# BurntSushi/aho-corasick

Hardware: NVIDIA H100
Metric: haystack_scan_throughput (higher is better)
Workload: dtype u8

## Files before the change

### aho-corasick_b200/csrc/acb_api.cu

```cuda
#include <cuda_runtime.h>

#include <algorithm>
#include <chrono>
#include <cstdio>
#include <cstdlib>
#include <cstring>
#include <atomic>
#include <pthread.h>
#include <condition_variable>
#include <functional>
#include <mutex>
#include <thread>
#include <new>
#include <optional>
#include <vector>

#include "../../include/acb200.h"
#include "../../include/acb200_debug.h"
#include "acb_build.hpp"
#include "acb_comm.hpp"
#include "acb_device.cuh"
#include "acb_plan.hpp"

using acb::DfaDev;
// ... 324 lines not shown
  d.pattern_lens = a->d_plens;
  d.depth16 = a->d_depth16;
  d.stride2 = h.stride2;
  d.max_match_id = h.max_match_id;
  d.start_unanchored_id = h.start_unanchored_id;
  d.start_anchored_id = h.start_anchored_id;
  d.max_pattern_len = uint32_t(std::min<uint64_t>(h.max_pattern_len, UINT32_MAX));
  d.min_pattern_len = uint32_t(std::min<uint64_t>(h.min_pattern_len, UINT32_MAX));
  d.amap = a->d_amap;
  acb::plan_device_fields(a->pf, d);
  a->on_device = true;
  return ACG_OK;
}

int reserve_tuples(Workspace& w, uint64_t cap) {
  return reserve_all(cap, w.d_keys[0], w.d_pids[0], w.d_keys[1], w.d_pids[1]);
}

template <class F>
int cub_call(Workspace& w, F f) {
  size_t tb = 0;
  CK(f(nullptr, tb));
  int rc = w.d_temp.reserve(std::max<size_t>(tb, 16));
  if (rc) return rc;
  tb = w.d_temp.cap;
  CK(f(w.d_temp, tb));
  return ACG_OK;
}

int reserve_rec(Workspace& w, uint64_t n) {
  n = std::max<uint64_t>(n, 1 << 16) * 3;
  int rc = w.d_rec.reserve(n);
  return rc ? rc : w.h_rec.reserve(n);
}

int reserve_docs(Workspace& w, uint64_t n) {
  return reserve_all(std::max<uint64_t>(n, 1 << 12), w.d_doc_offs, w.d_doc_counts, w.d_doc_incl, w.d_doc_flags);
}

int check_anchored(int have, int want_anchored) {
  if (have == ACG_START_BOTH) return ACG_OK;
  if (have == ACG_START_UNANCHORED) return want_anchored ? ACG_E_INVALID_INPUT_ANCHORED : ACG_OK;
  return want_anchored ? ACG_OK : ACG_E_INVALID_INPUT_UNANCHORED;
}
bool span_ok(uint64_t hay_len, uint64_t s, uint64_t e) { return e <= hay_len && s <= e + 1; }
int check_start(const HostDfa& h, int anchored) {
  if (anchored) return h.start_anchored_id == 0 ? ACG_E_INVALID_INPUT_ANCHORED : ACG_OK;
  return h.start_unanchored_id == 0 ? ACG_E_INVALID_INPUT_UNANCHORED : ACG_OK;
}

struct TupleResult {
  uint64_t n = 0;
  int sorted_buf = 0;
};

struct DocBatch {
  const uint64_t* d_offsets = nullptr;
  uint64_t n = 0;
  bool unordered = false;
};

struct BucketPlan {
  uint32_t shift = 0;
  uint32_t n = 0, log = 0, tie_bits = 0;
  uint64_t slots() const { return uint64_t(n) << log; }
};

BucketPlan plan_buckets(const acg_dfa* a, uint64_t n_bytes) {
  BucketPlan b;
  if (a->experiment & ACG_EXP_GLOBAL_TILES) return b;
  const uint32_t tie_bits = uint32_t(acb::bit_width(a->h.max_pattern_len)) + a->pf.dup_shift;
  if (tie_bits >= 32) return b;
  const uint32_t max_shift = 32 - tie_bits;
  uint32_t shift = std::min<uint32_t>(25, max_shift);
  uint32_t min_shift = 22;
  uint32_t log = acb::kOrderLog;
#ifdef ACB_EMULATE
  if (const char* e = getenv("ACB_EMU_BUCKETSHIFT")) { shift = std::min<uint32_t>(uint32_t(atoi(e)), max_shift); min_shift = 1; }
  if (const char* e = getenv("ACB_EMU_BUCKETLOG")) log = std::min<uint32_t>(uint32_t(std::max(atoi(e), 0)), acb::kOrderLog);
#endif
  if (shift < min_shift) return b;
  while ((n_bytes >> shift) + 1 > acb::kMaxBuckets) {
    if (shift >= max_shift) return b;
    ++shift;
  }
  b.shift = shift;
  b.n = uint32_t((n_bytes >> shift) + 1);
  b.log = log;
  b.tie_bits = tie_bits;
  return b;
}

int enqueue_prefilter_range(const acg_dfa* a, const uint8_t* d_hay, uint64_t readable,
                            uint64_t span_start, uint64_t span_end, uint64_t scan_lo,
                            uint64_t scan_hi, int mode, int dev_sms, const BucketPlan& bp,
                            const DocBatch* docs) {
  Workspace& w = cur_ws();
  const acb::PrefilterPlan& pf = a->pf;
  const uintptr_t base = reinterpret_cast<uintptr_t>(d_hay);
  uint64_t lo = scan_lo + ((16 - ((base + scan_lo) & 15)) & 15);
  const uint64_t limit = std::min<uint64_t>(scan_hi, readable >= 20 ? readable - 20 : 0);
  uint64_t hi = lo;
  if (limit > lo) hi = lo + ((limit - lo) & ~15ull);
  if (lo > scan_hi) { lo = scan_hi; hi = scan_hi; }
  acb::PrefilterLaunch p;
  p.hay = d_hay;
  p.hay_len = readable;
  p.span_start = span_start;
  p.span_end = span_end;
  p.bitmap = a->d_bitmap;
  p.log_bits = pf.log_bits;
  p.k = pf.k;
  p.stride = pf.stride;
  p.geom = pf.wide ? 1 : 0;
  p.dyn = (a->experiment & ACG_EXP_STATIC_TILES) ? 0 : ((a->experiment & ACG_EXP_GLOBAL_TILES) ? 2 : 1);
  p.kmask = pf.kmask;
  p.fold = pf.fold;
  p.mult = pf.mult;
  p.mult3 = pf.mult3;
  p.key_shift = pf.key_shift;
  p.shift = pf.shift;
  p.dense = pf.dense ? 1 : 0;
  p.brute = pf.brute ? 1 : 0;
  p.mode = mode == 1 ? 1 : 0;
  p.first_only = mode == 2 ? 1 : 0;
  p.dup_shift = pf.dup_shift;
  p.scan_lo = scan_lo;
  p.scan_hi = scan_hi;
  p.region_lo = lo;
  p.region_hi = hi;
  p.keys = w.d_keys[0];
  p.pids = w.d_pids[0];
  p.counter = w.d_counter;
  p.cap = w.tuple_cap();
  p.bucket_shift = bp.shift;
  p.bucket_log = bp.log;
  p.bucket_slots = bp.slots();
  p.doc_offsets = docs ? docs->d_offsets : nullptr;
  p.n_docs = docs ? docs->n : 0;
  p.bs_n = 0;
  for (int i = 0; i < 3; ++i) { p.bs_needle[i] = 0; p.bs_back[i] = 0; }
  if (pf.bs_n && !a->bytescan_inert && !(a->experiment & ACG_EXP_NO_BYTESCAN)) {
    p.bs_n = pf.bs_n;
    for (uint32_t i = 0; i < pf.bs_n; ++i) { p.bs_needle[i] = uint32_t(pf.bs_byte[i]) * 0x01010101u; p.bs_back[i] = pf.bs_back[i]; }
    CK(acb::launch_bytescan(a->dev, p, dev_sms, w.stream));
  } else {
    if (p.dyn == 2) CK(cudaMemsetAsync(w.d_counter + 2, 0, 8, w.stream));
    CK(acb::launch_prefilter(a->dev, p, dev_sms, w.stream));
  }
  cur_ws().stats.launches += 1;
  return ACG_OK;
}

int order_tuples(const acg_dfa* a, uint64_t want, uint64_t n_bytes, TupleResult* res, const BucketPlan& bp,
                 uint64_t overflow) {
  Workspace& w = cur_ws();
  res->n = want;
  cur_ws().stats.raw_matches = want;
  res->sorted_buf = 0;
  if (want <= 1 && (bp.shift == 0 || want == 0)) return ACG_OK;
  const int end_bit = std::min(64, acb::kTieBits + acb::bit_width(n_bytes + 1));
  float ms = 0;
  CK(cudaEventRecord(w.ev2, w.stream));
  auto sort_list = [&](int from) {
    return cub_call(w, [&](void* t, size_t& tb) {
      return acb::sort_pairs(t, tb, w.d_keys[from], w.d_keys[1 - from], w.d_pids[from], w.d_pids[1 - from], want,
                             end_bit, w.stream);
    });
  };
  int rc;
  if (bp.shift == 0) {
    if ((rc = sort_list(0))) return rc;
    cur_ws().stats.launches += 8;
    res->sorted_buf = 1;
  } else {
    acb::OrderLaunch o;
    o.keys_in = w.d_keys[0];
    o.pids_in = w.d_pids[0];
    o.keys_out = w.d_keys[1];
    o.pids_out = w.d_pids[1];
    o.bucket_count = w.d_counter + acb::kBucketCountersAt;
    o.overflow_count = w.d_counter;
    o.n_buckets = bp.n;
    o.bucket_shift = bp.shift;
    o.bucket_cap = 1u << bp.log;
    o.tie_bits = bp.tie_bits;
    o.bucket_slots = bp.slots();
    if (overflow == 0) {
      CK(acb::launch_order_buckets(o, w.stream));
      cur_ws().stats.launches += 1;
      res->sorted_buf = 1;
    } else {
      CK(acb::launch_compact_buckets(o, w.stream));
      if ((rc = sort_list(1))) return rc;
      cur_ws().stats.launches += 9;
      res->sorted_buf = 0;
    }
  }
  CK(cudaEventRecord(w.ev3, w.stream));
  CK(cudaStreamSynchronize(w.stream));
  cudaEventElapsedTime(&ms, w.ev2, w.ev3);
  cur_ws().stats.order_ms = ms;
  return ACG_OK;
}

int run_walk_overlapping(const acg_dfa* a, const uint8_t* d_hay, uint64_t readable, uint64_t span_start,
                         uint64_t span_end, TupleResult* res) {
  Workspace& w = cur_ws();
  const uint64_t n_bytes = span_end - span_start;
  if (a->max_list_len >= (1u << acb::kTieBits)) return ACG_E_INVALID_ARG;
  if (n_bytes >= (1ull << (64 - acb::kTieBits))) return ACG_E_INVALID_ARG;
  int dev_sms = 132;
  cudaDeviceGetAttribute(&dev_sms, cudaDevAttrMultiProcessorCount, a->device);
  const uint64_t target_lanes = uint64_t(dev_sms) * 2048;
  uint64_t seg_len = (n_bytes + target_lanes - 1) / std::max<uint64_t>(target_lanes, 1);
  seg_len = std::max<uint64_t>(seg_len, 256);
  seg_len = (seg_len + 15) & ~15ull;
  const uint64_t n_segs = std::max<uint64_t>((n_bytes + seg_len - 1) / seg_len, 1);
  uint64_t cap = std::max<uint64_t>(w.tuple_cap(), std::max<uint64_t>(1 << 20, n_bytes / 256));
  for (int attempt = 0; attempt < 8; ++attempt) {
    int rc = reserve_tuples(w, cap);
    if (rc) return rc;
    CK(cudaMemsetAsync(w.d_counter, 0, 8, w.stream));
    acb::WalkLaunch p;
    p.hay = d_hay;
    p.hay_len = readable;
    p.span_start = span_start;
    p.span_end = span_end;
    p.seg_len = seg_len;
    p.n_segs = n_segs;
    p.keys = w.d_keys[0];
    p.pids = w.d_pids[0];
    p.counter = w.d_counter;
    p.cap = w.tuple_cap();
    CK(cudaEventRecord(w.ev0, w.stream));
    CK(acb::launch_walk_overlapping(a->dev, p, w.stream));
    CK(cudaEventRecord(w.ev1, w.stream));
    CK(cudaMemcpyAsync(w.h_counter, w.d_counter, 8, cudaMemcpyDeviceToHost, w.stream));
    CK(cudaStreamSynchronize(w.stream));
    cur_ws().stats.launches += 1;
    const uint64_t want = *w.h_counter;
    if (want > w.tuple_cap()) { cap = want + want / 8 + 1024; continue; }
    float ms = 0;
    cudaEventElapsedTime(&ms, w.ev0, w.ev1);
    cur_ws().stats.scan_ms = ms;
    return order_tuples(a, want, n_bytes, res, BucketPlan{}, 0);
  }
  return ACG_E_NOMEM;
}

class CopyPool {
 public:
  static CopyPool& get() {
    static std::once_flag once;
    std::call_once(once, [] { pthread_atfork(nullptr, nullptr, [] { instance().store(nullptr); }); });
    CopyPool* p = instance().load(std::memory_order_acquire);
    if (!p) {
      CopyPool* fresh = new CopyPool;
      if (instance().compare_exchange_strong(p, fresh)) p = fresh;
    }
    return *p;
  }
  void copy(uint8_t* dst, const uint8_t* src, size_t n) {
    if (n < (4u << 20) || workers_.empty()) { std::memcpy(dst, src, n); return; }
    std::unique_lock<std::mutex> lk(mu_);
    busy_cv_.wait(lk, [&] { return !active_; });
    active_ = true;
    dst_ = dst; src_ = src; n_ = n;
    next_.store(0);
    pending_ = int(workers_.size());
    ++epoch_;
    cv_.notify_all();
    done_cv_.wait(lk, [&] { return pending_ == 0; });
    active_ = false;
    busy_cv_.notify_one();
  }

 private:
  static std::atomic<CopyPool*>& instance() {
    static std::atomic<CopyPool*> p{nullptr};
    return p;
  }
  CopyPool() {
    unsigned n = std::thread::hardware_concurrency();
    n = n >= 16 ? 8 : (n >= 4 ? n / 2 : 0);
    for (unsigned i = 0; i < n; ++i) workers_.emplace_back([this] { run(); });
    for (auto& t : workers_) t.detach();
  }
  void run() {
    uint64_t seen = 0;
    for (;;) {
      std::unique_lock<std::mutex> lk(mu_);
      cv_.wait(lk, [&] { return epoch_ != seen; });
      seen = epoch_;
      uint8_t* dst = dst_;
      const uint8_t* src = src_;
      const size_t n = n_;
      lk.unlock();
      constexpr size_t kSlice = 1u << 20;
      for (;;) {
        const size_t off = next_.fetch_add(kSlice);
        if (off >= n) break;
        std::memcpy(dst + off, src + off, std::min(kSlice, n - off));
      }
      lk.lock();
      if (--pending_ == 0) done_cv_.notify_one();
    }
  }
  std::mutex mu_;
  std::condition_variable cv_, done_cv_, busy_cv_;
  std::vector<std::thread> workers_;
  uint8_t* dst_ = nullptr;
  const uint8_t* src_ = nullptr;
  size_t n_ = 0;
  std::atomic<size_t> next_{0};
  int pending_ = 0;
  uint64_t epoch_ = 0;
  bool active_ = false;
};

bool is_pageable_host(const void* p) {
  cudaPointerAttributes attr;
  if (cudaPointerGetAttributes(&attr, p) != cudaSuccess) { cudaGetLastError(); return false; }
  return attr.type == cudaMemoryTypeUnregistered;
}

int reserve_stage(Workspace& w, uint64_t bytes) {
  for (int i = 0; i < 2; ++i) {
    int rc = w.h_stage[i].reserve(bytes);
    if (rc) return rc;
    if (!w.stage_ev[i]) CK(cudaEventCreateWithFlags(&w.stage_ev[i], cudaEventDisableTiming));
  }
  return ACG_OK;
}

int run_prefilter(const acg_dfa* a, const uint8_t* d_hay, uint64_t readable, uint64_t span_start,
                  uint64_t span_end, int mode, TupleResult* res, const uint8_t* h_hay = nullptr,
                  uint64_t scan_lo = UINT64_MAX, uint64_t scan_hi = UINT64_MAX, const DocBatch* docs = nullptr) {
  if (scan_lo == UINT64_MAX) { scan_lo = span_start; scan_hi = span_end; }
  const bool unordered = docs && docs->unordered;
  Workspace& w = cur_ws();
  const uint64_t n_bytes = span_end - span_start;
  if (n_bytes >= (1ull << (64 - acb::kTieBits))) return ACG_E_INVALID_ARG;
  int dev_sms = 132;
  cudaDeviceGetAttribute(&dev_sms, cudaDevAttrMultiProcessorCount, a->device);
  uint64_t cap = std::max<uint64_t>(w.tuple_cap(), std::max<uint64_t>(1 << 20, (scan_hi - scan_lo) / 256));
  const BucketPlan bp = unordered ? BucketPlan{} : plan_buckets(a, n_bytes);
  cap = std::max<uint64_t>(cap, bp.slots() + (bp.shift ? (1u << 16) : 0));
  const size_t counter_bytes = bp.shift ? 8 * (acb::kBucketCountersAt + size_t(bp.n)) : 16;
  bool copied = h_hay == nullptr;
  for (int attempt = 0; attempt < 8; ++attempt) {
    int rc = reserve_tuples(w, cap);
    if (rc) return rc;
    CK(cudaMemsetAsync(w.d_counter, 0, counter_bytes, w.stream));
    CK(cudaEventRecord(w.ev0, w.stream));
    if (copied) {
      if ((rc = enqueue_prefilter_range(a, d_hay, readable, span_start, span_end, scan_lo, scan_hi, mode,
                                        dev_sms, bp, docs)))
        return rc;
    } else {
      const uint64_t chunk = a->pipeline_chunk;
      const uint64_t tail = std::min<uint64_t>(a->h.max_pattern_len, 1u << 30) + 64;
      uint64_t scanned = span_start;
      const bool staged = span_end - span_start >= std::min<uint64_t>(8u << 20, chunk) && is_pageable_host(h_hay + span_start);
      if (staged && (rc = reserve_stage(w, std::min<uint64_t>(chunk, span_end - span_start)))) return rc;
      bool stage_used[2] = {false, false};
      int stage_i = 0;
      CK(cudaEventRecord(w.ev2, w.copy_stream));
      for (uint64_t c0 = span_start; c0 < span_end; c0 += chunk) {
        const uint64_t c1 = std::min(span_end, c0 + chunk);
        const uint8_t* src = h_hay + c0;
        if (staged) {
          if (stage_used[stage_i]) CK(cudaEventSynchronize(w.stage_ev[stage_i]));
          CopyPool::get().copy(w.h_stage[stage_i], h_hay + c0, size_t(c1 - c0));
          src = w.h_stage[stage_i];
        }
        CK(cudaMemcpyAsync(const_cast<uint8_t*>(d_hay) + c0, src, c1 - c0, cudaMemcpyHostToDevice,
                           w.copy_stream));
        if (staged) {
          CK(cudaEventRecord(w.stage_ev[stage_i], w.copy_stream));
          stage_used[stage_i] = true;
          stage_i ^= 1;
        }
        CK(cudaEventRecord(w.ev3, w.copy_stream));
        CK(cudaStreamWaitEvent(w.stream, w.ev3, 0));
        const uint64_t upto = c1 == span_end ? span_end : (c1 > scanned + tail ? c1 - tail : scanned);
        if (upto > scanned || c1 == span_end) {
          if ((rc = enqueue_prefilter_range(a, d_hay, c1 == span_end ? readable : c1, span_start, span_end,
                                            scanned, upto, mode, dev_sms, bp, docs)))
            return rc;
          scanned = upto;
        }
      }
      copied = true;
    }
    CK(cudaEventRecord(w.ev1, w.stream));
    CK(cudaMemcpyAsync(w.h_counter, w.d_counter, counter_bytes, cudaMemcpyDeviceToHost, w.stream));
    CK(cudaStreamSynchronize(w.stream));
    uint64_t want = w.h_counter[0], overflow = 0, room = w.tuple_cap();
    if (bp.shift) {
      overflow = want;
      want = 0;
      for (uint32_t i = 0; i < bp.n; ++i) want += w.h_counter[acb::kBucketCountersAt + i];
      room = w.tuple_cap() - bp.slots();
    }
    cur_ws().stats.candidates = w.h_counter[1];
    if (a->pf.bs_n && !a->bytescan_inert && scan_hi - scan_lo >= (1u << 16) && w.h_counter[1] > (scan_hi - scan_lo) / 64)
      a->bytescan_inert = true;
    float ms = 0;
    cudaEventElapsedTime(&ms, w.ev0, w.ev1);
    cur_ws().stats.scan_ms = ms;
    if (bp.shift ? overflow > room : want > w.tuple_cap()) {
      const uint64_t need = bp.shift ? overflow : want;
      cap = (w.tuple_cap() - room) + need + need / 8 + 1024;
      continue;
    }
    if (unordered) {
      res->n = want;
      res->sorted_buf = 0;
      cur_ws().stats.raw_matches = want;
      return ACG_OK;
    }
    return order_tuples(a, want, n_bytes, res, bp, overflow);
  }
  return ACG_E_NOMEM;
}

acb::TupleList tuple_list(const acg_dfa* a, const Workspace& w, const TupleResult& r) {
  return acb::TupleList{w.d_keys[r.sorted_buf], w.d_pids[r.sorted_buf], a->d_plens, r.n};
}

int run_chain(const acg_dfa* a, int mode, TupleResult* r) {
  Workspace& w = cur_ws();
  if (r->n == 0) return ACG_OK;
  int rc = reserve_all(std::max<uint64_t>(r->n, 1 << 16), w.d_scratch, w.d_flags);
  if (rc) return rc;
  const int dst = 1 - r->sorted_buf;
  acb::ChainLaunch c;
  c.t = tuple_list(a, w, *r);
  c.mode = mode;
  c.scratch_end = w.d_scratch;
  c.flags = w.d_flags;
  CK(cudaEventRecord(w.ev2, w.stream));
  CK(cudaMemsetAsync(w.d_flags, 0, r->n, w.stream));
  CK(acb::launch_chain_ends(c, w.stream));
  if ((rc = cub_call(w, [&](void* t, size_t& tb) { return acb::scan_max_u64(t, tb, w.d_scratch, r->n, w.stream); })))
    return rc;
  CK(acb::launch_chain_select(c, w.stream));
  if ((rc = cub_call(w, [&](void* t, size_t& tb) {
         return acb::select_flagged(t, tb, c.t.keys, c.t.pids, w.d_flags, w.d_keys[dst], w.d_pids[dst], w.d_counter,
                                    r->n, w.stream);
       })))
    return rc;
  CK(cudaEventRecord(w.ev3, w.stream));
  CK(cudaMemcpyAsync(w.h_counter, w.d_counter, 8, cudaMemcpyDeviceToHost, w.stream));
  CK(cudaStreamSynchronize(w.stream));
  float ms = 0;
  cudaEventElapsedTime(&ms, w.ev2, w.ev3);
  cur_ws().stats.order_ms += ms;
  cur_ws().stats.launches += 8;
  r->n = *w.h_counter;
  r->sorted_buf = dst;
  return ACG_OK;
}

int copy_out(uint64_t n, acg_match* out, uint64_t* fnv) {
  Workspace& w = cur_ws();
  if (n) CK(cudaMemcpyAsync(w.h_rec, w.d_rec, n * 24, cudaMemcpyDeviceToHost, w.stream));
  CK(cudaEventRecord(w.ev1, w.stream));
  CK(cudaStreamSynchronize(w.stream));
  float ms = 0;
  cudaEventElapsedTime(&ms, w.ev0, w.ev1);
  w.stats.d2h_ms += ms;
  if (fnv) {
    uint64_t hsh = 0xcbf29ce484222325ull;
    for (uint64_t i = 0; i < n * 3; ++i)
      for (int k = 0; k < 8; ++k) { hsh ^= (w.h_rec[i] >> (8 * k)) & 0xFF; hsh *= 0x100000001b3ull; }
    *fnv = hsh;
  } else if (n) {
    CopyPool::get().copy(reinterpret_cast<uint8_t*>(out), reinterpret_cast<const uint8_t*>(w.h_rec.p), n * 24);
  }
  return ACG_OK;
}

int run_seq(const acg_dfa* a, const uint8_t* d_hay, uint64_t span_start, uint64_t span_end,
            int anchored, int earliest, int single, acg_match* out, uint64_t cap, uint64_t* n_out) {
  Workspace& w = cur_ws();
  uint64_t scap = cap;
  int rc = reserve_docs(w, 2);
  if (rc) return rc;
  const uint64_t bounds[2] = {span_start, span_end};
  CK(cudaMemcpyAsync(w.d_doc_offs, bounds, sizeof(bounds), cudaMemcpyHostToDevice, w.stream));
  for (int attempt = 0; attempt < 4; ++attempt) {
    if ((rc = reserve_rec(w, scap))) return rc;
    acb::SeqDocsLaunch p{};
    p.hay = d_hay;
    p.doc_offsets = w.d_doc_offs;
    p.n_docs = 1;
    p.anchored = anchored;
    p.match_kind = a->h.match_kind;
    p.earliest = earliest;
    p.single = single;
    p.counts = w.d_counter;
    p.out = w.d_rec;
    p.cap = w.d_rec.cap / 3;
    CK(cudaEventRecord(w.ev0, w.stream));
    CK(acb::launch_seq_docs(a->dev, p, w.stream));
    CK(cudaEventRecord(w.ev1, w.stream));
    CK(cudaMemcpyAsync(w.h_counter, w.d_counter, 8, cudaMemcpyDeviceToHost, w.stream));
    CK(cudaStreamSynchronize(w.stream));
    cur_ws().stats.launches += 1;
    float ms = 0;
    cudaEventElapsedTime(&ms, w.ev0, w.ev1);
    cur_ws().stats.scan_ms = ms;
    const uint64_t n = *w.h_counter;
    *n_out = n;
    cur_ws().stats.raw_matches = n;
    if (n > cap) return ACG_E_OVERFLOW;
    if (n > w.d_rec.cap / 3) { scap = n; continue; }
    if (n) {
      CK(cudaMemcpyAsync(w.h_rec, w.d_rec, n * 24, cudaMemcpyDeviceToHost, w.stream));
      CK(cudaStreamSynchronize(w.stream));
      for (uint64_t i = 0; i < n; ++i) {
        out[i].pid = uint32_t(w.h_rec[i * 3]);
        out[i]._pad = 0;
        out[i].start = span_start + w.h_rec[i * 3 + 1];
        out[i].end = span_start + w.h_rec[i * 3 + 2];
      }
    }
    return ACG_OK;
  }
  return ACG_E_NOMEM;
}

int stage_host_span(const acg_dfa* a, const uint8_t* hay, uint64_t span_start, uint64_t span_end,
                    const uint8_t** d_base, bool alloc_only = false) {
  Workspace& w = cur_ws();
  const uint64_t lead = span_start & 15;
  const uint64_t bytes = span_end - span_start;
  const uint64_t need = bytes + lead + 64;
  if (need > w.d_hay.cap) {
    int rc = w.d_hay.reserve(((need + (1ull << 20)) >> 20) << 20);
    if (rc) return rc;
  }
  *d_base = w.d_hay + lead - span_start;
  if (alloc_only) return ACG_OK;
  CK(cudaEventRecord(w.ev0, w.stream));
  if (bytes)
    CK(cudaMemcpyAsync(w.d_hay + lead, hay + span_start, bytes, cudaMemcpyHostToDevice, w.stream));
  CK(cudaEventRecord(w.ev1, w.stream));
  CK(cudaStreamSynchronize(w.stream));
  float ms = 0;
  cudaEventElapsedTime(&ms, w.ev0, w.ev1);
  cur_ws().stats.h2d_ms = ms;
  return ACG_OK;
}

struct Placement {
  const uint8_t* base = nullptr;
  uint64_t readable = 0;
  const uint8_t* h_src = nullptr;
};

int place_input(const acg_dfa* a, const uint8_t* hay, bool on_device, uint64_t hay_len, uint64_t span_start,
                uint64_t span_end, bool pipelined, Placement* p) {
  if (on_device) {
    p->base = hay;
    p->readable = hay_len;
    return ACG_OK;
  }
  p->readable = span_end + 32;
  if (pipelined) p->h_src = hay;
  return stage_host_span(a, hay, span_start, span_end, &p->base, pipelined);
}

int find_earliest(const acg_dfa* a, int anchored, int earliest) {
// ... 1945 lines not shown
```

### aho-corasick_b200/csrc/acb_prefilter.cu

```cuda
#include "acb_device.cuh"
#include "acb_fingerprint.cuh"
#ifndef ACB_PTX_HEADER
#define ACB_PTX_HEADER "acb_ptx.cuh"
#endif
#include ACB_PTX_HEADER

#include <cstdio>
#include <cstdlib>
#include <type_traits>

#include <cub/device/device_scan.cuh>
#include <cub/device/device_select.cuh>

namespace acb {
namespace {

enum : int { kGeomNarrow = 0, kGeomWide = 1 };
template <int GEOM> struct PfGeom {
  static constexpr int kThreads = GEOM == kGeomNarrow ? 1024 : 512;
  static constexpr int kWarps = kThreads / 32;
  static constexpr int kGroups = GEOM == kGeomNarrow ? 2 : 4;
  static constexpr int kTile = kGroups * 512;
  static constexpr int kStageBytes = kTile + 16;
  static constexpr int kMinCtas = GEOM == kGeomWide ? 2 : 1;
  static constexpr uint32_t kLogBits = GEOM == kGeomWide ? kWideLogBits : kNarrowLogBits;
};
template <bool DENSE> struct PfCfg {
  static constexpr int kSlots = 256;
  static constexpr int kQ2 = DENSE ? 64 : 96;
};

#ifdef ACB_EMULATE
static const uint32_t kWinShift = getenv("ACB_EMU_WINSHIFT") ? (uint32_t)atoi(getenv("ACB_EMU_WINSHIFT")) : 31u;
#else
constexpr uint32_t kWinShift = 31;
#endif

constexpr int kPfStages = 2;

template <int GEOM, int STRIDE> struct PfPass {
  static constexpr bool kPair = STRIDE == 2 && GEOM == kGeomNarrow;
  static constexpr int kStages = kPair ? 1 : kPfStages;
  static constexpr int kGroups = PfGeom<GEOM>::kGroups * (kPair ? 2 : 1);
  static constexpr int kTile = kGroups * 512;
  static_assert(kStages * (kTile + 16) <= kPfStages * PfGeom<GEOM>::kStageBytes, "a step's tiles fit the warp's ring");
};

template <bool BUCKETED = true>
struct Emitter {
  uint64_t* g_keys;
  uint32_t* g_pids;
  unsigned long long* g_counter;
  uint64_t cap;
  uint32_t bucket_shift, bucket_log;
  uint64_t bucket_slots;
  __device__ __forceinline__ void emit(uint64_t key, uint32_t pid) {
    const unsigned m = __activemask();
    const int leader = __ffs(m) - 1;
    const int lane = threadIdx.x & 31;
    const bool bucketed = BUCKETED && bucket_shift != 0;
    unsigned long long* cnt = g_counter;
    uint64_t first = 0;
    bool together = true;
    if (bucketed) {
      const uint32_t b = (uint32_t)(key >> (kTieBits + bucket_shift));
      cnt += kBucketCountersAt + b;
      first = (uint64_t)b << bucket_log;
      together = __ballot_sync(m, b == (uint32_t)__shfl_sync(m, b, leader)) == m;
    }
    unsigned long long g;
    if (together) {
      unsigned long long base = 0;
      if (lane == leader) base = atomicAdd(cnt, (unsigned long long)__popc(m));
      base = __shfl_sync(m, base, leader);
      g = base + __popc(m & ((1u << lane) - 1));
    } else {
      g = atomicAdd(cnt, 1ull);
    }
    uint64_t slot = first + g;
    if (bucketed && g >> bucket_log) slot = bucket_slots + atomicAdd(g_counter, 1ull);
    if (slot < cap) { g_keys[slot] = key; g_pids[slot] = pid; }
  }
};

__device__ __forceinline__ uint32_t anchor_lookup_key(const DfaDev& d, uint32_t key) {
  uint32_t slot = amap_slot(key, d.amap_shift);
  for (;;) {
    const uint2 e = __ldg(d.amap + slot);
    if (e.y == 0 || e.x == key) return e.y;
    slot = amap_next(slot, d.amap_mask);
  }
}

__device__ __forceinline__ uint32_t anchor_lookup(const DfaDev& d, const PrefilterLaunch& p, uint64_t s) {
  if (s + d.amap_k > p.span_end) return 0;
  const uintptr_t a = reinterpret_cast<uintptr_t>(p.hay + s);
  const uintptr_t lo_edge = reinterpret_cast<uintptr_t>(p.hay), hi_edge = lo_edge + p.hay_len;
  const uintptr_t wa = a & ~uintptr_t(3);
  uint32_t key;
  if (wa >= lo_edge && wa + ((a & 3) ? 8 : 4) <= hi_edge) {
    const uint32_t* w = reinterpret_cast<const uint32_t*>(wa);
    const uint32_t lo = __ldg(w);
    const uint32_t hi = (a & 3) ? __ldg(w + 1) : 0u;
    key = __funnelshift_r(lo, hi, (uint32_t)(a & 3) * 8) & d.amap_kmask;
  } else {
    key = 0;
    for (uint32_t i = 0; i < d.amap_k; ++i) key |= (uint32_t)__ldg(p.hay + s + i) << (8 * i);
  }
  return anchor_lookup_key(d, key);
}

__device__ __forceinline__ uint64_t doc_end_of(const uint64_t* __restrict__ offs, uint64_t n_docs, uint64_t s) {
  uint64_t lo = 1, hi = n_docs;
  while (lo < hi) {
    const uint64_t mid = lo + ((hi - lo) >> 1);
    if (__ldg(offs + mid) > s) hi = mid; else lo = mid + 1;
  }
  return __ldg(offs + lo);
}

template <int MODE, class EM>
__device__ __forceinline__ void verify_from(const DfaDev& d, const PrefilterLaunch& p, const uint8_t* s_cls,
                                            uint64_t s, uint32_t sid, uint32_t j, EM& em) {
  const uint8_t* __restrict__ hay = p.hay;
  const uint32_t* __restrict__ trans = d.trans;
  uint64_t pos = s + j;
  uint32_t best_pid = 0, best_len = 0;
  bool entered = j != 0;
  for (;;) {
    if (!entered) {
      if (pos >= p.span_end) break;
      const uint32_t b = __ldg(hay + pos);
      sid = __ldg(trans + sid + s_cls[b]);
      ++j;
      ++pos;
      if (sid == 0) break;
      if (__ldg(d.depth16 + (sid >> d.stride2)) != j) break;
    }
    entered = false;
    if (sid <= d.max_match_id) {
      if (p.doc_offsets != nullptr && pos > doc_end_of(p.doc_offsets, p.n_docs, s)) break;
      const uint32_t row = sid >> d.stride2;
      const uint32_t lo = __ldg(d.match_offsets + row - 2), hi = __ldg(d.match_offsets + row - 1);
      if (MODE == 0) {
        for (uint32_t i = lo; i < hi; ++i) {
          const uint32_t pid = __ldg(d.match_pids + i);
          if (__ldg(d.pattern_lens + pid) != j) break;
          if (p.first_only && i > lo) break;
          const uint64_t tie = ((uint64_t)(d.max_pattern_len - j) << p.dup_shift) | (uint64_t)(i - lo);
          em.emit(((pos - p.span_start) << kTieBits) | tie, pid);
        }
      } else {
        const uint32_t pid = __ldg(d.match_pids + lo);
        if (__ldg(d.pattern_lens + pid) == j) { best_pid = pid; best_len = j; }
      }
    }
  }
  if (MODE == 1 && best_len) em.emit(((s - p.span_start) << kTieBits) | best_len, best_pid);
}

template <int MODE, class EM>
// ... 453 lines not shown
  auto load = [&](uint64_t base) -> uint4 {
    return base < load_end ? ptx::ld_nc_u4(p.hay + base) : make_uint4(0, 0, 0, 0);
  };
  auto process = [&](uint64_t base, const uint4& v) {
    const bool in_range = base < load_end;
    const uint32_t w[4] = {v.x, v.y, v.z, v.w};
    uint32_t zany = 0;
#pragma unroll
    for (int j = 0; j < 3; ++j) {
      if (j >= (int)n_needles) break;
      const uint32_t needle = p.bs_needle[j];
#pragma unroll
      for (int k = 0; k < 4; ++k) {
        const uint32_t x = w[k] ^ needle;
        zany |= (x - 0x01010101u) & ~x & 0x80808080u;
      }
    }
    if (!__any_sync(0xffffffffu, zany != 0 && in_range)) return;
    uint32_t cand = 0;
#pragma unroll
    for (int j = 0; j < 3; ++j) {
      if (j >= (int)n_needles) break;
      const uint32_t needle = p.bs_needle[j];
      uint32_t m = 0;
#pragma unroll
      for (int k = 0; k < 4; ++k) {
        const uint32_t x = w[k] ^ needle;
        const uint32_t z = (x - 0x01010101u) & ~x & 0x80808080u;
        m |= ((((z >> 7) * 0x00204081u) >> 21) & 0xFu) << (4 * k);
      }
      if (!in_range) m = 0;
      const uint32_t back = p.bs_back[j];
      if (back == 0) {
        cand |= m;
      } else {
        const uint32_t both = m | (__shfl_down_sync(0xffffffffu, m, 1) << 16);
        uint32_t smear = both;
        for (uint32_t sft = 1; sft <= back; ++sft) smear |= both >> sft;
        cand |= smear & 0xFFFFu;
      }
    }
    if (lane >= (int)owned_lanes || base >= p.region_hi) cand = 0;
    const uint32_t cnt = __popc(cand);
    if (__any_sync(0xffffffffu, cnt != 0)) {
      uint32_t slot = 0, total = 0;
#pragma unroll
      for (int b = 0; b < 5; ++b) {
        const uint32_t bl = __ballot_sync(0xffffffffu, (cnt >> b) & 1u);
        slot += __popc(bl & lt) << b;
        total += __popc(bl) << b;
      }
      if (qlen + total > (uint32_t)kBsQueue) drain();
      if (total > (uint32_t)kBsQueue) {
        uint32_t c = cand, nver = 0;
        while (c) {
          const int bit = __ffs(c) - 1;
          c &= c - 1;
          verify_at<MODE>(d, p, s_cls, base + bit, em);
          ++nver;
        }
        cand_total += __reduce_add_sync(0xffffffffu, nver);
      } else {
        uint64_t* dst = q + qlen + slot;
        uint32_t c = cand;
        while (c) {
          const int bit = __ffs(c) - 1;
          c &= c - 1;
          *dst++ = base + bit;
        }
        qlen += total;
        if (qlen >= 64) drain();
      }
    }
  };
  const uint64_t stride = (uint64_t)gridDim.x * kBsWarps;
  auto base_of = [&](uint64_t st) { return p.region_lo + st * step_bytes + (uint64_t)lane * 16; };
  uint64_t st = (uint64_t)blockIdx.x * kBsWarps + warp;
  uint4 cur[2], nxt[2];
#pragma unroll
  for (int u = 0; u < 2; ++u) cur[u] = st + u * stride < n_steps ? load(base_of(st + u * stride)) : make_uint4(0, 0, 0, 0);
  for (; st < n_steps; st += 2 * stride) {
#pragma unroll
    for (int u = 0; u < 2; ++u) {
      const uint64_t sn = st + (2 + u) * stride;
      nxt[u] = sn < n_steps ? load(base_of(sn)) : make_uint4(0, 0, 0, 0);
    }
#pragma unroll
    for (int u = 0; u < 2; ++u)
      if (st + u * stride < n_steps) process(base_of(st + u * stride), cur[u]);
    cur[0] = nxt[0];
    cur[1] = nxt[1];
  }
  if (qlen) drain();
  if (lane == 0 && cand_total) atomicAdd(p.counter + 1, cand_total);
}


__device__ __forceinline__ void tuple_span(const ChainLaunch& c, uint64_t i, uint64_t* s, uint64_t* e) {
  const uint64_t key = c.t.keys[i];
  if (c.mode == 1) {
    *s = key >> kTieBits;
    *e = *s + (key & kTieMask);
  } else {
    *e = key >> kTieBits;
    *s = *e - c.t.pattern_lens[c.t.pids[i]];
  }
}

__global__ void chain_ends_kernel(ChainLaunch c) {
  const uint64_t i = (uint64_t)blockIdx.x * blockDim.x + threadIdx.x;
  if (i >= c.t.n) return;
  uint64_t s, e;
  tuple_span(c, i, &s, &e);
  c.scratch_end[i] = e;
}

__global__ void chain_select_kernel(ChainLaunch c) {
  const uint64_t i = (uint64_t)blockIdx.x * blockDim.x + threadIdx.x;
  if (i >= c.t.n) return;
  uint64_t s, e;
  tuple_span(c, i, &s, &e);
  if (i > 0 && c.scratch_end[i - 1] > s) return;
  c.flags[i] = 1;
  uint64_t cur_end = e;
  for (uint64_t j = i + 1; j < c.t.n; ++j) {
    uint64_t sj, ej;
    tuple_span(c, j, &sj, &ej);
    if (c.scratch_end[j - 1] <= sj) break;
    if (sj >= cur_end) { c.flags[j] = 1; cur_end = ej; } else c.flags[j] = 0;
  }
}

struct MaxOp {
  __device__ __forceinline__ uint64_t operator()(uint64_t a, uint64_t b) const { return a > b ? a : b; }
};

constexpr int kOrdThreads = 1024;
constexpr int kOrdWarps = kOrdThreads / 32;
constexpr int kOrdRounds = (int)kOrderCap / kOrdThreads;
constexpr int kOrdBatch = 8;

__global__ void __launch_bounds__(kOrdThreads, 1) order_buckets_kernel(OrderLaunch o) {
  ACB_DYNAMIC_SMEM(smem_raw);
  const uint32_t cap = o.bucket_cap;
  uint32_t* ka = reinterpret_cast<uint32_t*>(smem_raw);
  uint32_t* kb = ka + cap;
  uint16_t* ia = reinterpret_cast<uint16_t*>(kb + cap);
  uint16_t* ib = ia + cap;
  uint16_t* s_cnt = ib + cap;
  uint32_t* s_sum = reinterpret_cast<uint32_t*>(s_cnt + 256 * kOrdWarps);
  const int tid = threadIdx.x, lane = tid & 31, warp = tid >> 5;
  const uint32_t lt = (1u << lane) - 1;
  const uint32_t b = blockIdx.x;
  const uint32_t n = (uint32_t)o.bucket_count[b];
  if (n == 0) return;

  uint32_t part = 0;
  for (uint32_t i = tid; i < b; i += kOrdThreads) part += (uint32_t)o.bucket_count[i];
  part = __reduce_add_sync(0xffffffffu, part);
  if (lane == 0) s_sum[warp] = part;
  __syncthreads();
  uint64_t out0 = 0;
  for (int w = 0; w < kOrdWarps; ++w) out0 += s_sum[w];

  const uint64_t in0 = (uint64_t)b * cap;
  const uint64_t off0 = (uint64_t)b << o.bucket_shift;
  const uint32_t tie_bits = o.tie_bits;
  const uint64_t tie_mask = (1ull << tie_bits) - 1;
  for (uint32_t j0 = 0; j0 < n; j0 += kOrdBatch * kOrdThreads) {
    uint64_t k[kOrdBatch];
#pragma unroll
    for (int u = 0; u < kOrdBatch; ++u) {
      const uint32_t j = j0 + u * kOrdThreads + tid;
      k[u] = j < n ? o.keys_in[in0 + j] : 0;
    }
#pragma unroll
    for (int u = 0; u < kOrdBatch; ++u) {
      const uint32_t j = j0 + u * kOrdThreads + tid;
      if (j < n) {
        ka[j] = (uint32_t)((((k[u] >> kTieBits) - off0) << tie_bits) | (k[u] & tie_mask));
        ia[j] = (uint16_t)j;
      }
    }
  }

  const uint32_t per_warp = (n + kOrdWarps - 1) / kOrdWarps;
  const uint32_t w_lo = min(warp * per_warp, n), w_hi = min(w_lo + per_warp, n);
  const uint32_t rounds = (per_warp + 31) / 32;
  const uint32_t key_bits = o.bucket_shift + tie_bits;
  for (uint32_t sh = 0; sh < key_bits; sh += 8) {
    for (int i = tid; i < 256 * kOrdWarps / 2; i += kOrdThreads) reinterpret_cast<uint32_t*>(s_cnt)[i] = 0;
    __syncthreads();
    uint32_t rd[kOrdRounds];
#pragma unroll
    for (int r = 0; r < kOrdRounds; ++r) {
      rd[r] = 0;
      if ((uint32_t)r < rounds) {
        const uint32_t i = w_lo + r * 32 + lane;
        const bool valid = i < w_hi;
        const uint32_t digit = valid ? (ka[i] >> sh) & 0xFFu : 0u;
        uint32_t peers = __ballot_sync(0xffffffffu, valid);
#pragma unroll
        for (int bit = 0; bit < 8; ++bit) {
          const uint32_t bb = __ballot_sync(0xffffffffu, (digit >> bit) & 1u);
          peers &= ((digit >> bit) & 1u) ? bb : ~bb;
        }
        uint16_t* c = s_cnt + digit * kOrdWarps + warp;
        const uint32_t base = valid ? *c : 0u;
        __syncwarp();
        if (valid && (peers & lt) == 0) *c = (uint16_t)(base + __popc(peers));
        __syncwarp();
        rd[r] = (digit << 16) | (base + __popc(peers & lt));
      }
    }
    __syncthreads();
    {
      constexpr int kPer = 256 * kOrdWarps / kOrdThreads;
      uint16_t* c = s_cnt + tid * kPer;
      uint32_t v[kPer], sum = 0;
#pragma unroll
      for (int u = 0; u < kPer; ++u) { v[u] = c[u]; sum += v[u]; }
      uint32_t incl = sum;
#pragma unroll
      for (int d = 1; d < 32; d <<= 1) {
        const uint32_t x = (uint32_t)__shfl_sync(0xffffffffu, incl, lane >= d ? lane - d : lane);
        if (lane >= d) incl += x;
      }
      if (lane == 31) s_sum[warp] = incl;
      __syncthreads();
      uint32_t run = incl - sum;
      for (int w = 0; w < warp; ++w) run += s_sum[w];
#pragma unroll
      for (int u = 0; u < kPer; ++u) { c[u] = (uint16_t)run; run += v[u]; }
    }
    __syncthreads();
#pragma unroll
    for (int r = 0; r < kOrdRounds; ++r) {
      const uint32_t i = w_lo + r * 32 + lane;
      if ((uint32_t)r < rounds && i < w_hi) {
        const uint32_t dst = s_cnt[(rd[r] >> 16) * kOrdWarps + warp] + (rd[r] & 0xFFFFu);
        kb[dst] = ka[i];
        ib[dst] = ia[i];
      }
    }
    __syncthreads();
    uint32_t* tk = ka; ka = kb; kb = tk;
    uint16_t* ti = ia; ia = ib; ib = ti;
  }

  for (uint32_t j0 = 0; j0 < n; j0 += kOrdBatch * kOrdThreads) {
    uint32_t pid[kOrdBatch];
#pragma unroll
    for (int u = 0; u < kOrdBatch; ++u) {
      const uint32_t j = j0 + u * kOrdThreads + tid;
      pid[u] = j < n ? o.pids_in[in0 + ia[j]] : 0u;
    }
#pragma unroll
    for (int u = 0; u < kOrdBatch; ++u) {
      const uint32_t j = j0 + u * kOrdThreads + tid;
      if (j < n) {
        const uint32_t sk = ka[j];
        o.keys_out[out0 + j] = ((off0 + (sk >> tie_bits)) << kTieBits) | (sk & tie_mask);
        o.pids_out[out0 + j] = pid[u];
      }
    }
  }
}

constexpr int kCompactThreads = 256;
__global__ void __launch_bounds__(kCompactThreads) compact_buckets_kernel(OrderLaunch o) {
  __shared__ unsigned long long s_part[kCompactThreads];
  const uint32_t b = blockIdx.x;
  const int tid = threadIdx.x;
  unsigned long long part = 0;
  for (uint32_t i = tid; i < b && i < o.n_buckets; i += kCompactThreads) part += min(o.bucket_count[i], (unsigned long long)o.bucket_cap);
  s_part[tid] = part;
  __syncthreads();
  uint64_t dst = 0;
  for (int i = 0; i < kCompactThreads; ++i) dst += s_part[i];
  const uint64_t n = b < o.n_buckets ? min(o.bucket_count[b], (unsigned long long)o.bucket_cap) : *o.overflow_count;
  const uint64_t src = b < o.n_buckets ? (uint64_t)b * o.bucket_cap : o.bucket_slots;
  for (uint64_t j = tid; j < n; j += kCompactThreads) {
    o.keys_out[dst + j] = o.keys_in[src + j];
    o.pids_out[dst + j] = o.pids_in[src + j];
  }
}

}

cudaError_t launch_prefilter(const DfaDev& dfa, const PrefilterLaunch& p, int sm_count, cudaStream_t s) {
  const bool dense = p.dense != 0;
  const int geom = p.stride == 2 ? p.geom : kGeomNarrow;
  if (geom < kGeomNarrow || geom > kGeomWide) return cudaErrorInvalidValue;
  const uint32_t want_log = geom == kGeomWide ? PfGeom<kGeomWide>::kLogBits : PfGeom<kGeomNarrow>::kLogBits;
  if (!p.brute && (p.log_bits != want_log || p.shift != bloom_shift(want_log))) return cudaErrorInvalidValue;
  const size_t bitmap_bytes = p.brute ? 0 : (size_t(1) << (p.log_bits - 3));
  static const int kThreadsOf[2] = {PfGeom<0>::kThreads, PfGeom<1>::kThreads};
  static const int kStageOf[2] = {PfGeom<0>::kStageBytes, PfGeom<1>::kStageBytes};
  const int threads = kThreadsOf[geom];
  const int warps = threads / 32;
  const int stage_bytes = kStageOf[geom];
  const int tile = geom == kGeomWide ? PfPass<kGeomWide, 2>::kTile
                   : p.stride == 2 ? PfPass<kGeomNarrow, 2>::kTile : PfPass<kGeomNarrow, 1>::kTile;
  const int q2_bytes = dense ? PfCfg<true>::kQ2 * 8 : PfCfg<false>::kQ2 * 4;
  const int slot_bytes = PfCfg<false>::kSlots * 2;
  const size_t smem = size_t(warps) * (kPfStages * stage_bytes + kPfStages * 12 + q2_bytes + slot_bytes) + 16 + bitmap_bytes;
  if (smem > 227 * 1024 - 1024) return cudaErrorInvalidValue;
  const bool masked = p.fold != 0 || p.kmask != 0xFFFFFFFFu;
  using KernT = void (*)(DfaDev, PrefilterLaunch);
#define ACB_PF_ROW(M, K, D)                                                                                 \
  {prefilter_kernel<M, K, false, 1, kGeomNarrow, D>, prefilter_kernel<M, K, true, 1, kGeomNarrow, D>, \
   prefilter_kernel<M, K, false, 2, kGeomNarrow, D>, prefilter_kernel<M, K, false, 2, kGeomWide, D>}
  static const KernT table[2][2][3][4] = {
      {{ACB_PF_ROW(0, false, 0), ACB_PF_ROW(0, false, 1), ACB_PF_ROW(0, false, 2)},
       {ACB_PF_ROW(0, true, 0), ACB_PF_ROW(0, true, 1), ACB_PF_ROW(0, true, 2)}},
      {{ACB_PF_ROW(1, false, 0), ACB_PF_ROW(1, false, 1), ACB_PF_ROW(1, false, 2)},
       {ACB_PF_ROW(1, true, 0), ACB_PF_ROW(1, true, 1), ACB_PF_ROW(1, true, 2)}}};
#undef ACB_PF_ROW
  if (p.dyn > 2) return cudaErrorInvalidValue;
  if (p.stride == 2 && dense) return cudaErrorInvalidValue;
  int variant = dense ? 1 : 0;
  if (p.stride == 2) variant = geom == kGeomWide ? 3 : 2;
  KernT kern = table[p.mode ? 1 : 0][masked ? 1 : 0][p.dyn][variant];
#ifdef ACB_EMULATE
  if (getenv("ACB_EMU_TRACE")) fprintf(stderr, "launch_prefilter variant %d dyn %d threads %d smem %zu\n", variant, (int)p.dyn, threads, smem);
#endif
  cudaError_t e = cudaFuncSetAttribute(kern, cudaFuncAttributeMaxDynamicSharedMemorySize, (int)smem);
  if (e != cudaSuccess) return e;
  int per_sm = 1;
  e = cudaOccupancyMaxActiveBlocksPerMultiprocessor(&per_sm, kern, threads, smem);
  if (e != cudaSuccess) return e;
  if (per_sm < 1) per_sm = 1;
  uint64_t grid = (uint64_t)sm_count * per_sm;
  const uint64_t cta_step = uint64_t(warps) * tile;
  const uint64_t warp_steps = ((p.region_hi - p.region_lo) + cta_step - 1) / cta_step;
  if (grid > warp_steps) grid = warp_steps ? warp_steps : 1;
  ACB_LAUNCH(kern, (unsigned)grid, threads, smem, s, dfa, p);
  return cudaGetLastError();
}

cudaError_t launch_bytescan(const DfaDev& dfa, const PrefilterLaunch& p, int sm_count, cudaStream_t s) {
  if (p.bs_n < 1 || p.bs_n > 3) return cudaErrorInvalidValue;
  for (uint32_t j = 0; j < 3; ++j)
    if (p.bs_back[j] > 15) return cudaErrorInvalidValue;
  uint64_t grid = (uint64_t)sm_count * 2;
  const uint64_t steps = ((p.region_hi - p.region_lo) + 16 * 31 - 1) / (16 * 31);
  const uint64_t ctas = (steps + kBsWarps - 1) / kBsWarps;
  if (grid > ctas) grid = ctas ? ctas : 1;
  if (p.mode) ACB_LAUNCH(bytescan_kernel<1>, (unsigned)grid, kBsThreads, 0, s, dfa, p);
  else ACB_LAUNCH(bytescan_kernel<0>, (unsigned)grid, kBsThreads, 0, s, dfa, p);
  return cudaGetLastError();
}

cudaError_t launch_chain_ends(const ChainLaunch& c, cudaStream_t s) {
  const unsigned blocks = (unsigned)((c.t.n + 255) / 256);
  ACB_LAUNCH(chain_ends_kernel, blocks, 256, 0, s, c);
  return cudaGetLastError();
}
cudaError_t launch_chain_select(const ChainLaunch& c, cudaStream_t s) {
  const unsigned blocks = (unsigned)((c.t.n + 255) / 256);
  ACB_LAUNCH(chain_select_kernel, blocks, 256, 0, s, c);
  return cudaGetLastError();
}
cudaError_t launch_order_buckets(const OrderLaunch& o, cudaStream_t s) {
  if (o.n_buckets == 0 || o.n_buckets > kMaxBuckets || o.bucket_cap == 0 || o.bucket_cap > kOrderCap ||
      o.bucket_shift + o.tie_bits > 32)
    return cudaErrorInvalidValue;
  const size_t smem = size_t(o.bucket_cap) * 12 + 256 * kOrdWarps * 2 + kOrdWarps * 4;
  cudaError_t e = cudaFuncSetAttribute(order_buckets_kernel, cudaFuncAttributeMaxDynamicSharedMemorySize, (int)smem);
  if (e != cudaSuccess) return e;
  ACB_LAUNCH(order_buckets_kernel, o.n_buckets, kOrdThreads, smem, s, o);
  return cudaGetLastError();
}
cudaError_t launch_compact_buckets(const OrderLaunch& o, cudaStream_t s) {
  ACB_LAUNCH(compact_buckets_kernel, o.n_buckets + 1, kCompactThreads, 0, s, o);
  return cudaGetLastError();
}
cudaError_t scan_max_u64(void* d_temp,size_t& temp_bytes, uint64_t* data, uint64_t n, cudaStream_t s) {
  return cub::DeviceScan::InclusiveScan(d_temp, temp_bytes, data, data, MaxOp(), (int64_t)n, s);
}
cudaError_t select_flagged(void* d_temp, size_t& temp_bytes, const uint64_t* keys_in, const uint32_t* pids_in,
                           const uint8_t* flags, uint64_t* keys_out, uint32_t* pids_out,
                           unsigned long long* d_num_out, uint64_t n, cudaStream_t s) {
  size_t a = 0, b = 0;
  if (d_temp == nullptr) {
    cudaError_t e = cub::DeviceSelect::Flagged(nullptr, a, keys_in, flags, keys_out, d_num_out, (int64_t)n, s);
    if (e != cudaSuccess) return e;
    e = cub::DeviceSelect::Flagged(nullptr, b, pids_in, flags, pids_out, d_num_out, (int64_t)n, s);
    temp_bytes = a > b ? a : b;
    return e;
  }
  cudaError_t e = cub::DeviceSelect::Flagged(d_temp, temp_bytes, keys_in, flags, keys_out, d_num_out, (int64_t)n, s);
  if (e != cudaSuccess) return e;
  return cub::DeviceSelect::Flagged(d_temp, temp_bytes, pids_in, flags, pids_out, d_num_out, (int64_t)n, s);
}

}
```

Baseline: 2160.

## Queue bucket ordering before host sync and cache kernel attribute setup

The bucket-ordering kernel is now enqueued on the stream right after the scan, before the host reads back counters. The kernel itself checks the device-side overflow counter and exits early if it is nonzero, so the host no longer needs a sync followed by a separate launch when there is no overflow. Separately, cudaFuncSetAttribute and occupancy queries are memoized per kernel, smem size and device behind a mutex, which avoids repeated driver calls on every launch. The risk is wasted bucket-kernel blocks launched when overflow occurs, plus a global lock on the launch path.

```diff
diff --git a/aho-corasick_b200/csrc/acb_api.cu b/aho-corasick_b200/csrc/acb_api.cu
--- a/aho-corasick_b200/csrc/acb_api.cu
+++ b/aho-corasick_b200/csrc/acb_api.cu
@@ -500,8 +500,23 @@
   return ACG_OK;
 }
 
-int order_tuples(const acg_dfa* a, uint64_t want, uint64_t n_bytes, TupleResult* res, const BucketPlan& bp,
-                 uint64_t overflow) {
+acb::OrderLaunch order_launch(const Workspace& w, const BucketPlan& bp) {
+  acb::OrderLaunch o;
+  o.keys_in = w.d_keys[0];
+  o.pids_in = w.d_pids[0];
+  o.keys_out = w.d_keys[1];
+  o.pids_out = w.d_pids[1];
+  o.bucket_count = w.d_counter + acb::kBucketCountersAt;
+  o.overflow_count = w.d_counter;
+  o.n_buckets = bp.n;
+  o.bucket_shift = bp.shift;
+  o.bucket_cap = 1u << bp.log;
+  o.tie_bits = bp.tie_bits;
+  o.bucket_slots = bp.slots();
+  return o;
+}
+
+int order_tuples(const acg_dfa* a, uint64_t want, uint64_t n_bytes, TupleResult* res, const BucketPlan& bp) {
   Workspace& w = cur_ws();
   res->n = want;
   cur_ws().stats.raw_matches = want;
@@ -522,28 +537,10 @@
     cur_ws().stats.launches += 8;
     res->sorted_buf = 1;
   } else {
-    acb::OrderLaunch o;
-    o.keys_in = w.d_keys[0];
-    o.pids_in = w.d_pids[0];
-    o.keys_out = w.d_keys[1];
-    o.pids_out = w.d_pids[1];
-    o.bucket_count = w.d_counter + acb::kBucketCountersAt;
-    o.overflow_count = w.d_counter;
-    o.n_buckets = bp.n;
-    o.bucket_shift = bp.shift;
-    o.bucket_cap = 1u << bp.log;
-    o.tie_bits = bp.tie_bits;
-    o.bucket_slots = bp.slots();
-    if (overflow == 0) {
-      CK(acb::launch_order_buckets(o, w.stream));
-      cur_ws().stats.launches += 1;
-      res->sorted_buf = 1;
-    } else {
-      CK(acb::launch_compact_buckets(o, w.stream));
-      if ((rc = sort_list(1))) return rc;
-      cur_ws().stats.launches += 9;
-      res->sorted_buf = 0;
-    }
+    CK(acb::launch_compact_buckets(order_launch(w, bp), w.stream));
+    if ((rc = sort_list(1))) return rc;
+    cur_ws().stats.launches += 9;
+    res->sorted_buf = 0;
   }
   CK(cudaEventRecord(w.ev3, w.stream));
   CK(cudaStreamSynchronize(w.stream));
@@ -592,7 +589,7 @@
     float ms = 0;
     cudaEventElapsedTime(&ms, w.ev0, w.ev1);
     cur_ws().stats.scan_ms = ms;
-    return order_tuples(a, want, n_bytes, res, BucketPlan{}, 0);
+    return order_tuples(a, want, n_bytes, res, BucketPlan{});
   }
   return ACG_E_NOMEM;
 }
@@ -743,6 +740,13 @@
       copied = true;
     }
     CK(cudaEventRecord(w.ev1, w.stream));
+    const bool queued = bp.shift != 0;
+    if (queued) {
+      CK(cudaEventRecord(w.ev2, w.stream));
+      CK(acb::launch_order_buckets(order_launch(w, bp), w.stream));
+      cur_ws().stats.launches += 1;
+      CK(cudaEventRecord(w.ev3, w.stream));
+    }
     CK(cudaMemcpyAsync(w.h_counter, w.d_counter, counter_bytes, cudaMemcpyDeviceToHost, w.stream));
     CK(cudaStreamSynchronize(w.stream));
     uint64_t want = w.h_counter[0], overflow = 0, room = w.tuple_cap();
@@ -769,7 +773,15 @@
       cur_ws().stats.raw_matches = want;
       return ACG_OK;
     }
-    return order_tuples(a, want, n_bytes, res, bp, overflow);
+    if (queued && overflow == 0) {
+      res->n = want;
+      res->sorted_buf = 1;
+      cur_ws().stats.raw_matches = want;
+      cudaEventElapsedTime(&ms, w.ev2, w.ev3);
+      cur_ws().stats.order_ms = ms;
+      return ACG_OK;
+    }
+    return order_tuples(a, want, n_bytes, res, bp);
   }
   return ACG_E_NOMEM;
 }
diff --git a/aho-corasick_b200/csrc/acb_prefilter.cu b/aho-corasick_b200/csrc/acb_prefilter.cu
--- a/aho-corasick_b200/csrc/acb_prefilter.cu
+++ b/aho-corasick_b200/csrc/acb_prefilter.cu
@@ -7,6 +7,10 @@
 
 #include <cstdio>
 #include <cstdlib>
+#include <map>
+#include <mutex>
+#include <tuple>
+#include <utility>
 #include <type_traits>
 
 #include <cub/device/device_scan.cuh>
@@ -766,6 +770,7 @@
   const int tid = threadIdx.x, lane = tid & 31, warp = tid >> 5;
   const uint32_t lt = (1u << lane) - 1;
   const uint32_t b = blockIdx.x;
+  if (*o.overflow_count != 0) return;
   const uint32_t n = (uint32_t)o.bucket_count[b];
   if (n == 0) return;
 
@@ -898,6 +903,31 @@
     o.keys_out[dst + j] = o.keys_in[src + j];
     o.pids_out[dst + j] = o.pids_in[src + j];
   }
+}
+
+template <class K>
+cudaError_t kernel_setup(K kern, int threads, size_t smem, int* per_sm) {
+  static std::mutex mu;
+  static std::map<std::tuple<const void*, size_t, int>, int> known;
+  static std::map<std::pair<const void*, int>, size_t> limit;
+  int dev = 0;
+  cudaError_t e = cudaGetDevice(&dev);
+  if (e != cudaSuccess) return e;
+  const void* f = reinterpret_cast<const void*>(kern);
+  const auto key = std::make_tuple(f, smem, dev);
+  std::lock_guard<std::mutex> lk(mu);
+  const auto it = known.find(key);
+  if (it != known.end()) { *per_sm = it->second; return cudaSuccess; }
+  size_t& lim = limit[std::make_pair(f, dev)];
+  if (smem > lim) {
+    e = cudaFuncSetAttribute(kern, cudaFuncAttributeMaxDynamicSharedMemorySize, (int)smem);
+    if (e != cudaSuccess) return e;
+    lim = smem;
+  }
+  e = cudaOccupancyMaxActiveBlocksPerMultiprocessor(per_sm, kern, threads, smem);
+  if (e != cudaSuccess) return e;
+  known.emplace(key, *per_sm);
+  return cudaSuccess;
 }
 
 }
@@ -939,10 +969,8 @@
 #ifdef ACB_EMULATE
   if (getenv("ACB_EMU_TRACE")) fprintf(stderr, "launch_prefilter variant %d dyn %d threads %d smem %zu\n", variant, (int)p.dyn, threads, smem);
 #endif
-  cudaError_t e = cudaFuncSetAttribute(kern, cudaFuncAttributeMaxDynamicSharedMemorySize, (int)smem);
-  if (e != cudaSuccess) return e;
   int per_sm = 1;
-  e = cudaOccupancyMaxActiveBlocksPerMultiprocessor(&per_sm, kern, threads, smem);
+  cudaError_t e = kernel_setup(kern, threads, smem, &per_sm);
   if (e != cudaSuccess) return e;
   if (per_sm < 1) per_sm = 1;
   uint64_t grid = (uint64_t)sm_count * per_sm;
@@ -981,7 +1009,8 @@
       o.bucket_shift + o.tie_bits > 32)
     return cudaErrorInvalidValue;
   const size_t smem = size_t(o.bucket_cap) * 12 + 256 * kOrdWarps * 2 + kOrdWarps * 4;
-  cudaError_t e = cudaFuncSetAttribute(order_buckets_kernel, cudaFuncAttributeMaxDynamicSharedMemorySize, (int)smem);
+  int per_sm = 1;
+  cudaError_t e = kernel_setup(order_buckets_kernel, kOrdThreads, smem, &per_sm);
   if (e != cudaSuccess) return e;
   ACB_LAUNCH(order_buckets_kernel, o.n_buckets, kOrdThreads, smem, s, o);
   return cudaGetLastError();
```

After: 2164, median of 6. Within noise of the previous version (+0.2%).
